# varunagrawal/tiny-faces-pytorch

Measured on AMD Instinct MI355X. Metric: train img/s @ 500x500 bs=12/GPU, higher is better.
Workload: dtype bf16; 1 GPU; configs[2]: bs=12/GPU synthetic 500x500 crops + random boxes; dense_overlap targets on GPU, ResNet-101 hybrid-head fwd, criterion, bwd, fused SGD; global_batch=12, image=500x500, templates=25, parallelism=dp1, weights=random init (tamed kaiming), fp32 master + bf16 MFMA operands

## Files before the change

tiny-faces-pytorch_amd/csrc/common.h:

```cpp
#pragma once
#include <hip/hip_runtime.h>
#include <hip/hip_ext.h>
#include <stdint.h>

#include "../../include/tinyfaces_hip.h"

#define TF_LAUNCH_WITH_STOP_EVENT(kernel, grid, block, lds, stream, ...)                                                  \
  do {                                                                                                                  \
    hipEvent_t ev__ = tf::take_next_stop_event();                                                                       \
    if (ev__) hipExtLaunchKernelGGL(kernel, grid, block, lds, stream, nullptr, ev__, 0, __VA_ARGS__);                   \
    else hipLaunchKernelGGL(kernel, grid, block, lds, stream, __VA_ARGS__);                                             \
  } while (0)

#define TF_LAUNCH_TIMED(kernel, grid, block, lds, stream, ...)                                                            \
  do {                                                                                                                  \
    hipEvent_t f__ = tf::take_next_stop_event(), a__ = nullptr, b__ = nullptr;                                          \
    if (f__) {                                                                                                          \
      tf::ProfScope::fall_back_to_bracket();                                                                            \
      hipExtLaunchKernelGGL(kernel, grid, block, lds, stream, nullptr, f__, 0, __VA_ARGS__);                            \
    } else if (tf::ProfScope::take_launch_events(&a__, &b__)) {                                                         \
      hipExtLaunchKernelGGL(kernel, grid, block, lds, stream, a__, b__, 0, __VA_ARGS__);                                \
    } else {                                                                                                            \
      hipLaunchKernelGGL(kernel, grid, block, lds, stream, __VA_ARGS__);                                                \
    }                                                                                                                   \
  } while (0)

#define TF_CHECK_LAUNCH()                                  \
  do {                                                     \
    hipError_t e__ = hipGetLastError();                    \
    if (e__ != hipSuccess) return TF_ERR_LAUNCH;           \
  } while (0)

namespace tf {

void set_next_stop_event(hipEvent_t e);
hipEvent_t take_next_stop_event();

constexpr int kWave = 64;

__device__ __forceinline__ float bf16_to_f32(uint16_t h) { return __uint_as_float(((uint32_t)h) << 16); }
typedef __bf16 tf_bf16x2 __attribute__((ext_vector_type(2)));
typedef float tf_f32x2 __attribute__((ext_vector_type(2)));
__device__ __forceinline__ uint32_t pack_bf16x2(float lo, float hi) {
  return __builtin_bit_cast(uint32_t, __builtin_convertvector(tf_f32x2{lo, hi}, tf_bf16x2));
}
__device__ __forceinline__ uint16_t f32_to_bf16(float f) { return (uint16_t)(pack_bf16x2(f, 0.f) & 0xffffu); }

template <typename T> struct Elem;
template <> struct Elem<float> {
  static constexpr int kPer16B = 4;
  __device__ static __forceinline__ float load(const float* p) { return *p; }
  __device__ static __forceinline__ void store(float* p, float v) { *p = v; }
};
struct bf16_t { uint16_t v; };
template <> struct Elem<bf16_t> {
  static constexpr int kPer16B = 8;
  __device__ static __forceinline__ float load(const bf16_t* p) { return bf16_to_f32(p->v); }
  __device__ static __forceinline__ void store(bf16_t* p, float v) { p->v = f32_to_bf16(v); }
};

struct f16_t { uint16_t v; };
__device__ __forceinline__ float f16_to_f32(uint16_t h) { return (float)__builtin_bit_cast(_Float16, h); }
__device__ __forceinline__ uint16_t f32_to_f16(float f) { return __builtin_bit_cast(uint16_t, (_Float16)f); }
__device__ __forceinline__ uint32_t pack_f16x2(float lo, float hi) { return (uint32_t)f32_to_f16(lo) | ((uint32_t)f32_to_f16(hi) << 16); }
template <> struct Elem<f16_t> {
  static constexpr int kPer16B = 8;
  __device__ static __forceinline__ float load(const f16_t* p) { return f16_to_f32(p->v); }
  __device__ static __forceinline__ void store(f16_t* p, float v) { p->v = f32_to_f16(v); }
};
template <typename T> __device__ __forceinline__ uint32_t pack2(float lo, float hi);
template <> __device__ __forceinline__ uint32_t pack2<bf16_t>(float lo, float hi) { return pack_bf16x2(lo, hi); }
template <> __device__ __forceinline__ uint32_t pack2<f16_t>(float lo, float hi) { return pack_f16x2(lo, hi); }

template <typename T> __device__ __forceinline__ void unpack16(const uint4& r, float* f);
template <> __device__ __forceinline__ void unpack16<float>(const uint4& r, float* f) {
  f[0] = __uint_as_float(r.x); f[1] = __uint_as_float(r.y); f[2] = __uint_as_float(r.z); f[3] = __uint_as_float(r.w);
}
template <> __device__ __forceinline__ void unpack16<bf16_t>(const uint4& r, float* f) {
  f[0] = __uint_as_float(r.x << 16); f[1] = __uint_as_float(r.x & 0xffff0000u);
  f[2] = __uint_as_float(r.y << 16); f[3] = __uint_as_float(r.y & 0xffff0000u);
  f[4] = __uint_as_float(r.z << 16); f[5] = __uint_as_float(r.z & 0xffff0000u);
  f[6] = __uint_as_float(r.w << 16); f[7] = __uint_as_float(r.w & 0xffff0000u);
}
template <> __device__ __forceinline__ void unpack16<f16_t>(const uint4& r, float* f) {
  f[0] = f16_to_f32((uint16_t)r.x); f[1] = f16_to_f32((uint16_t)(r.x >> 16));
  f[2] = f16_to_f32((uint16_t)r.y); f[3] = f16_to_f32((uint16_t)(r.y >> 16));
  f[4] = f16_to_f32((uint16_t)r.z); f[5] = f16_to_f32((uint16_t)(r.z >> 16));
  f[6] = f16_to_f32((uint16_t)r.w); f[7] = f16_to_f32((uint16_t)(r.w >> 16));
}
template <typename T> __device__ __forceinline__ uint4 pack16(const float* f);
template <> __device__ __forceinline__ uint4 pack16<float>(const float* f) {
  return make_uint4(__float_as_uint(f[0]), __float_as_uint(f[1]), __float_as_uint(f[2]), __float_as_uint(f[3]));
}
template <> __device__ __forceinline__ uint4 pack16<bf16_t>(const float* f) {
  return make_uint4(pack_bf16x2(f[0], f[1]), pack_bf16x2(f[2], f[3]), pack_bf16x2(f[4], f[5]), pack_bf16x2(f[6], f[7]));
}

template <> __device__ __forceinline__ uint4 pack16<f16_t>(const float* f) {
  return make_uint4(pack_f16x2(f[0], f[1]), pack_f16x2(f[2], f[3]), pack_f16x2(f[4], f[5]), pack_f16x2(f[6], f[7]));
}

__device__ __forceinline__ double wave_sum(double v) {
#pragma unroll
  for (int o = 32; o > 0; o >>= 1) v += __shfl_xor(v, o, 64);
  return v;
}
template <int O> __device__ __forceinline__ float lane_xor_sum(float v) {
  if constexpr (O == 8) {
    return v + __int_as_float(__builtin_amdgcn_update_dpp(0, __float_as_int(v), 0x128 , 0xf, 0xf, false));
  } else if constexpr (O == 16) {
    typedef unsigned u32x2_ __attribute__((ext_vector_type(2)));
    const u32x2_ r = __builtin_amdgcn_permlane16_swap(__float_as_uint(v), __float_as_uint(v), false, false);
    return __uint_as_float(r.x) + __uint_as_float(r.y);
  } else if constexpr (O == 32) {
    typedef unsigned u32x2_ __attribute__((ext_vector_type(2)));
    const u32x2_ r = __builtin_amdgcn_permlane32_swap(__float_as_uint(v), __float_as_uint(v), false, false);
    return __uint_as_float(r.x) + __uint_as_float(r.y);
  } else {
    return v + __shfl_xor(v, O, 64);
  }
}
template <int FROM> __device__ __forceinline__ float lane_group_sum(float v) {
  if constexpr (FROM <= 32) { v = lane_xor_sum<FROM>(v); if constexpr (FROM < 32) v = lane_group_sum<FROM * 2>(v); }
  return v;
}
__device__ __forceinline__ float wave_sum(float v) {
  v += __int_as_float(__builtin_amdgcn_update_dpp(0, __float_as_int(v), 0x128, 0xf, 0xf, false));
  v += __int_as_float(__builtin_amdgcn_update_dpp(0, __float_as_int(v), 0x124, 0xf, 0xf, false));
  v += __int_as_float(__builtin_amdgcn_update_dpp(0, __float_as_int(v), 0x122, 0xf, 0xf, false));
  v += __int_as_float(__builtin_amdgcn_update_dpp(0, __float_as_int(v), 0x121, 0xf, 0xf, false));
  return lane_group_sum<16>(v);
}
__device__ __forceinline__ int lane_id() { return threadIdx.x & 63; }

__device__ __host__ __forceinline__ uint64_t mix64(uint64_t z) {
  z += 0x9e3779b97f4a7c15ull;
  z = (z ^ (z >> 30)) * 0xbf58476d1ce4e5b9ull;
  z = (z ^ (z >> 27)) * 0x94d049bb133111ebull;
  return z ^ (z >> 31);
}
__device__ __host__ __forceinline__ uint64_t hash4(uint64_t a, uint64_t b, uint64_t c, uint64_t d) {
  return mix64(mix64(mix64(mix64(a) ^ b) ^ c) ^ d);
}
__device__ __host__ __forceinline__ double u01(uint64_t h) { return (double)(h >> 11) * (1.0 / 9007199254740992.0); }


struct PerDevice {
  bool done[64] = {};
  bool first() { int dev = 0; (void)hipGetDevice(&dev); bool& d = done[dev & 63]; const bool f = !d; d = true; return f; }
};
inline int device_cus() {
  static int cus[64] = {};
  int dev = 0; (void)hipGetDevice(&dev);
  int& n = cus[dev & 63];
  if (n == 0) { int v = 0; if (hipDeviceGetAttribute(&v, hipDeviceAttributeMultiprocessorCount, dev) != hipSuccess || v <= 0) v = 256; n = v; }
  return n;
}

}
```

tiny-faces-pytorch_amd/csrc/targets.hip:

```cpp
#include "targets_shared.h"

namespace {

__device__ __forceinline__ double iou14(double x1, double y1, double x2, double y2, double farea,
                                        double gx1, double gy1, double gx2, double gy2) {
  double bw = gx2 - gx1 + 1.0, bh = gy2 - gy1 + 1.0;
  double barea = bw * bh;
  double xx1 = fmax(x1, gx1), yy1 = fmax(y1, gy1), xx2 = fmin(x2, gx2), yy2 = fmin(y2, gy2);
  double iw = xx2 - xx1 + 1.0, ih = yy2 - yy1 + 1.0;
  double ov = 0.0;
  if (ih > 0.0 && iw > 0.0) {
    double ia = iw * ih;
    double un = farea + barea - ia;
    ov = ia / un;
  }
  return rint(ov * 1e14) / 1e14;
}

__device__ __forceinline__ double noise_at(const TgtParams& p, int b, int flat, int g, int G) {
  if (p.noise) return p.noise[p.noise_off[b] + (int64_t)flat * G + g];
  return tf::u01(tf::hash4(p.seed, (uint64_t)b, (uint64_t)flat, (uint64_t)g));
}

__device__ __forceinline__ bool pad_at(const TgtParams& p, int b, int y, int x, double dx1, double dy1,
                                       double dx2, double dy2) {
  if (!p.paste) return false;
  int xs = (p.flips && p.flips[b]) ? (p.vsx - 1 - x) : x;
  double cx = (double)(p.ofx + xs * p.stx), cy = (double)(p.ofy + y * p.sty);
  const int32_t* pb = p.paste + 4 * b;
  return (cx + dx1 < (double)(pb[0] + 1)) | (cy + dy1 < (double)(pb[1] + 1)) |
         (cx + dx2 > (double)pb[2]) | (cy + dy2 > (double)pb[3]);
}

struct TgtCompParams : TgtParams {
  int32_t* own; double* best; int32_t* count; int32_t* match_count;
  int nslots, N; double T;
};
template <class P> struct is_comp { static constexpr bool value = false; };
template <> struct is_comp<TgtCompParams> { static constexpr bool value = true; };

template <int PHASE, class P = TgtParams>
__global__ void __launch_bounds__(256) targets_kernel(P p) {
  constexpr bool COMP = is_comp<P>::value;
  if constexpr (COMP) {
    if (p.box_off[gridDim.y] > p.nslots) return;
  }
  const int b = blockIdx.y;
  const int cells = p.vsy * p.vsx;
  const int idx = blockIdx.x * 256 + threadIdx.x;
  const bool active = idx < p.nt * cells;
  const int t = active ? idx / cells : 0;
  const int cell = active ? idx - t * cells : 0;
  const int y = cell / p.vsx, x = cell - y * p.vsx;
  const int flat = cell * p.nt + t;
  const int g0 = p.box_off[b], G = p.box_off[b + 1] - g0;
  const double* tp = p.tpl + (size_t)t * p.tstride;
  const double dx1 = tp[0], dy1 = tp[1], dx2 = tp[2], dy2 = tp[3];
  const Anchor an = anchor_at(dx1, dy1, dx2, dy2, p.ofy, p.ofx, p.sty, p.stx, y, x);
  const double fw = an.fw, fh = an.fh;

  double best = -1.0; int bestg = 0;
  for (int g = 0; g < G; ++g) {
    const double* bx = p.boxes + 4 * (size_t)(g0 + g);
    const double gx1 = bx[0], gy1 = bx[1], gx2 = bx[2], gy2 = bx[3];
    double v = -1.0;
    if (active) {
      double r = iou14(an.x1, an.y1, an.x2, an.y2, an.farea, gx1, gy1, gx2, gy2);
      v = r + 1e-6 * noise_at(p, b, flat, g, G);
      if (v > best) { best = v; bestg = g; }
    }
    const bool hot = v > p.neg_thresh;
    if (__ballot(hot)) {
      unsigned long long bits = hot ? (unsigned long long)__double_as_longlong(v) : 0ull;
      if (PHASE == 0) {
        unsigned long long m = bits;
#pragma unroll
        for (int o = 32; o > 0; o >>= 1) {
          unsigned long long other = __shfl_xor(m, o, 64);
          m = other > m ? other : m;
        }
        if (tf::lane_id() == 0) atomicMax(&p.gmax[g0 + g], m);
      } else {
        if (hot && bits == p.gmax[g0 + g]) atomicMin(&p.gidx[g0 + g], (unsigned int)flat);
      }
    }
  }
  if (PHASE != 0 || !active) return;

  float cls = -1.f, tx = 0.f, ty = 0.f, tw = 0.f, th = 0.f;
  if (G > 0) {
    const double* bx = p.boxes + 4 * (size_t)(g0 + bestg);
    const double gx1 = bx[0], gy1 = bx[1], gx2 = bx[2], gy2 = bx[3];
    const double fcx = (gx1 + gx2) / 2.0, fcy = (gy1 + gy2) / 2.0;
    const double coarse_x = (double)(p.ofx + x * p.stx), coarse_y = (double)(p.ofy + y * p.sty);
    tx = (float)((fcx - coarse_x) / fw);
    ty = (float)((fcy - coarse_y) / fh);
    tw = (float)log((gx2 - gx1 + 1.0) / fw);
    th = (float)log((gy2 - gy1 + 1.0) / fh);
    if (best >= p.pos_thresh) cls = 1.f;
    else if (p.neg_thresh <= best && best < p.pos_thresh) cls = 0.f;
  }
  if (cls != -1.f && pad_at(p, b, y, x, dx1, dy1, dx2, dy2)) { cls = 0.f; tx = 0.f; }
  const size_t plane = (size_t)cells;
  p.cls[((size_t)b * p.nt + t) * plane + cell] = cls;
  float* r = p.reg + ((size_t)b * 4 * p.nt + t) * plane + cell;
  r[0] = tx; r[(size_t)p.nt * plane] = ty; r[(size_t)2 * p.nt * plane] = tw; r[(size_t)3 * p.nt * plane] = th;
  if constexpr (COMP) {
    const size_t a = (size_t)b * p.nt * plane + idx;
    p.own[a] = bestg; p.best[a] = best;
  }
}

__global__ void targets_best_anchor_kernel(TgtParams p, int total) {
  int gi = blockIdx.x * blockDim.x + threadIdx.x;
  if (gi >= total) return;
  if (__longlong_as_double((long long)p.gmax[gi]) > p.neg_thresh) {
    const int b = image_of(p.box_off, gi);
    unsigned int flat = p.gidx[gi];
    int t = flat % p.nt, cell = flat / p.nt;
    int y = cell / p.vsx, x = cell - y * p.vsx;
    const double* tp = p.tpl + (size_t)t * p.tstride;
    if (!pad_at(p, b, y, x, tp[0], tp[1], tp[2], tp[3]))
      p.cls[((size_t)b * p.nt + t) * (size_t)(p.vsy * p.vsx) + cell] = 1.f;
  }
}


__global__ void __launch_bounds__(256) targets_count_kernel(TgtCompParams p) {
  if (p.box_off[gridDim.y] > p.nslots) return;
  const int b = blockIdx.y;
  const int A = p.nt * p.vsy * p.vsx;
  const int idx = blockIdx.x * 256 + threadIdx.x;
  int slot = -1;
  if (idx < A) {
    const size_t a = (size_t)b * A + idx;
    if (p.cls[a] == 1.f) slot = p.box_off[b] + p.own[a];
  }
  unsigned long long pending = __ballot(slot >= 0);
  while (pending) {
    const int leader = __ffsll((long long)pending) - 1;
    const int s = __shfl(slot, leader, 64);
    const unsigned long long same = __ballot(slot == s);
    if (tf::lane_id() == leader) atomicAdd(&p.count[s], (int)__popcll(same));
    pending &= ~same;
  }
}

__device__ __forceinline__ bool cand_before(unsigned long long ka, unsigned int fa, unsigned long long kb, unsigned int fb) {
  return ka > kb || (ka == kb && fa < fb);
}

__global__ void __launch_bounds__(256) targets_select_kernel(TgtCompParams p, int B) {
  __shared__ unsigned long long s_k[4];
  __shared__ unsigned int s_f[4];
  const int gi = blockIdx.x;
  const int total = p.box_off[B];
  if (total > p.nslots || gi >= total) return;
  const int cnt = p.count[gi];
  const int need = p.N - cnt;
  if (need <= 0) {
    if (threadIdx.x == 0 && p.match_count) p.match_count[gi] = cnt;
    return;
  }
  const int b = image_of(p.box_off, gi);
  const int g = gi - p.box_off[b];
  const double* bx = p.boxes + 4 * (size_t)gi;
  const double gx1 = bx[0], gy1 = bx[1], gx2 = bx[2], gy2 = bx[3];
  const int cells = p.vsy * p.vsx;
  const size_t img = (size_t)b * p.nt * cells;
  const int wave = threadIdx.x >> 6;
  const double bw = gx2 - gx1 + 1.0, bh = gy2 - gy1 + 1.0, barea = bw * bh;
  const double Tm = p.T - 2e-6;

  unsigned long long prev_k = ~0ull;
  unsigned int prev_f = 0;
  int promoted = 0;
  while (promoted < need) {
    unsigned long long my_k = 0ull;
    unsigned int my_f = 0xffffffffu;
    for (int t = wave; t < p.nt; t += 4) {
      const double* tp = p.tpl + (size_t)t * p.tstride;
      const double dx1 = tp[0], dy1 = tp[1], dx2 = tp[2], dy2 = tp[3];
      const double fw = dx2 - dx1 + 1.0, fh = dy2 - dy1 + 1.0, farea = fw * fh;
      const double larger = fmax(farea, barea);
      if (!(fmin(farea, barea) >= Tm * larger)) continue;
      const double iwm = Tm * larger / fmin(fh, bh) * (1.0 - 1e-9), ihm = Tm * larger / fmin(fw, bw) * (1.0 - 1e-9);
      const double xl = fmax(floor((gx1 - 1.0 + iwm - dx2 - (double)p.ofx) / (double)p.stx), 0.0);
      const double xh = fmin(ceil((gx2 + 1.0 - iwm - dx1 - (double)p.ofx) / (double)p.stx), (double)(p.vsx - 1));
      const double yl = fmax(floor((gy1 - 1.0 + ihm - dy2 - (double)p.ofy) / (double)p.sty), 0.0);
      const double yh = fmin(ceil((gy2 + 1.0 - ihm - dy1 - (double)p.ofy) / (double)p.sty), (double)(p.vsy - 1));
      if (!(xl <= xh) || !(yl <= yh)) continue;
      const int x0 = (int)xl, y0 = (int)yl, ww = (int)xh - x0 + 1, wh = (int)yh - y0 + 1;
      for (int i = tf::lane_id(); i < ww * wh; i += 64) {
        const int wy = i / ww;
        const int y = y0 + wy, x = x0 + (i - wy * ww);
        const int cell = y * p.vsx + x;
        const size_t a = img + (size_t)t * cells + cell;
        if (p.own[a] != g) continue;
        const double bv = p.best[a];
        if (!(bv >= p.T) || p.cls[a] == 1.f || pad_at(p, b, y, x, dx1, dy1, dx2, dy2)) continue;
        const unsigned long long k = (unsigned long long)__double_as_longlong(bv);
        const unsigned int f = (unsigned int)(cell * p.nt + t);
        if (cand_before(prev_k, prev_f, k, f) && cand_before(k, f, my_k, my_f)) { my_k = k; my_f = f; }
      }
    }
#pragma unroll
    for (int o = 32; o > 0; o >>= 1) {
      const unsigned long long ok = __shfl_xor(my_k, o, 64);
      const unsigned int of = __shfl_xor(my_f, o, 64);
      if (cand_before(ok, of, my_k, my_f)) { my_k = ok; my_f = of; }
    }
    if (tf::lane_id() == 0) { s_k[wave] = my_k; s_f[wave] = my_f; }
    __syncthreads();
    unsigned long long win_k = s_k[0];
    unsigned int win_f = s_f[0];
#pragma unroll
    for (int w = 1; w < 4; ++w)
      if (cand_before(s_k[w], s_f[w], win_k, win_f)) { win_k = s_k[w]; win_f = s_f[w]; }
    __syncthreads();
    if (win_k == 0ull) break;
    if (threadIdx.x == 0) {
      const int t = win_f % p.nt, cell = win_f / p.nt;
      p.cls[img + (size_t)t * cells + cell] = 1.f;
    }
    prev_k = win_k; prev_f = win_f;
    ++promoted;
  }
  if (threadIdx.x == 0 && p.match_count) p.match_count[gi] = cnt + promoted;
}

__global__ void iou_dump_kernel(const double* boxes, int G, const double* tpl, int nt, int tstride, int vsy, int vsx,
                                int ofy, int ofx, int sty, int stx, double* out) {
  int flat = blockIdx.x * blockDim.x + threadIdx.x;
  if (flat >= vsy * vsx * nt) return;
  int t = flat % nt, cell = flat / nt, y = cell / vsx, x = cell % vsx;
  const double* tp = tpl + (size_t)t * tstride;
  double cx = (double)ofx + (double)x * ((double)stx / 1.0), cy = (double)ofy + (double)y * ((double)sty / 1.0);
  double fh = tp[3] - tp[1] + 1.0, fw = tp[2] - tp[0] + 1.0;
  for (int g = 0; g < G; ++g)
    out[(size_t)flat * G + g] = iou14(tp[0] + cx, tp[1] + cy, tp[2] + cx, tp[3] + cy, fw * fh,
                                      boxes[4 * g], boxes[4 * g + 1], boxes[4 * g + 2], boxes[4 * g + 3]);
}

}

extern "C" size_t tf_targets_workspace_bytes(int total_boxes) {
  size_t n = (size_t)(total_boxes > 0 ? total_boxes : 1);
  return n * 8 + n * 4 + 64;
}

extern "C" int tf_dense_overlap_targets(const double* boxes, const int32_t* box_offsets, int B,
                                        const double* templates, int nt, int tstride,
                                        int vsy, int vsx, int ofy, int ofx, int sty, int stx,
                                        const int32_t* paste_boxes, const int32_t* flips,
                                        const double* noise, const int64_t* noise_offsets, uint64_t seed,
                                        double pos_thresh, double neg_thresh,
                                        float* class_map, float* reg_map,
                                        void* ws, size_t ws_bytes, void* stream_) {
  hipStream_t stream = (hipStream_t)stream_;
  TgtParams p;
  if (int rc = base_params(p, boxes, box_offsets, B, templates, nt, tstride, vsy, vsx, ofy, ofx, sty, stx, paste_boxes, flips, noise, noise_offsets,
                           seed, pos_thresh, neg_thresh, class_map, reg_map)) return rc;
  size_t nslots = (ws_bytes - 64) / 12;
  if (!ws || ws_bytes < 76) return TF_ERR_WORKSPACE;
  p.gmax = (unsigned long long*)ws;
  p.gidx = (unsigned int*)((char*)ws + nslots * 8);
  if (hipMemsetAsync(p.gmax, 0, nslots * 8, stream) != hipSuccess) return TF_ERR_LAUNCH;
  if (hipMemsetAsync(p.gidx, 0xff, nslots * 4, stream) != hipSuccess) return TF_ERR_LAUNCH;
  dim3 grid((nt * vsy * vsx + 255) / 256, B);
  hipLaunchKernelGGL(targets_kernel<0>, grid, dim3(256), 0, stream, p);
  hipLaunchKernelGGL(targets_kernel<1>, grid, dim3(256), 0, stream, p);
  int total = (int)nslots;
  hipLaunchKernelGGL(targets_best_anchor_kernel, dim3((total + 127) / 128), dim3(128), 0, stream, p, total);
  TF_CHECK_LAUNCH();
  return TF_OK;
}

extern "C" size_t tf_targets_comp_workspace_bytes(int total_boxes, int B, int nt, int vsy, int vsx) {
  size_t n = (size_t)(total_boxes > 0 ? total_boxes : 1);
  size_t anchors = (size_t)(B > 0 ? B : 0) * (size_t)(nt > 0 ? nt : 0) * (size_t)(vsy > 0 ? vsy : 0) * (size_t)(vsx > 0 ? vsx : 0);
  return n * 16 + anchors * 12 + 64;
}

extern "C" int tf_dense_overlap_targets_comp(const double* boxes, const int32_t* box_offsets, int B,
                                             const double* templates, int nt, int tstride,
                                             int vsy, int vsx, int ofy, int ofx, int sty, int stx,
                                             const int32_t* paste_boxes, const int32_t* flips,
                                             const double* noise, const int64_t* noise_offsets, uint64_t seed,
                                             double pos_thresh, double neg_thresh,
                                             int N, double T, int32_t* match_count,
                                             float* class_map, float* reg_map,
                                             void* ws, size_t ws_bytes, void* stream_) {
  hipStream_t stream = (hipStream_t)stream_;
  TgtCompParams p;
  if (int rc = base_params(p, boxes, box_offsets, B, templates, nt, tstride, vsy, vsx, ofy, ofx, sty, stx, paste_boxes, flips, noise, noise_offsets,
                           seed, pos_thresh, neg_thresh, class_map, reg_map)) return rc;
  if (sty <= 0 || stx <= 0) return TF_ERR_ARG;
  if (N < 1 || N > 64) return TF_ERR_ARG;
  if (!(T >= 0.01) || !(T < pos_thresh) || !(T - T == 0.0)) return TF_ERR_ARG;
  const size_t anchors = (size_t)B * nt * vsy * vsx;
  if ((size_t)nt * vsy * vsx > (size_t)0x7fffffff) return TF_ERR_UNSUPPORTED;
  if (!ws || ws_bytes < tf_targets_comp_workspace_bytes(1, B, nt, vsy, vsx)) return TF_ERR_WORKSPACE;
  size_t nslots = (ws_bytes - 64 - anchors * 12) / 16;
  if (nslots > ((size_t)1 << 30)) nslots = (size_t)1 << 30;
  char* w = (char*)ws;
  p.gmax = (unsigned long long*)w;                 w += nslots * 8;
  p.best = (double*)w;                             w += anchors * 8;
  p.gidx = (unsigned int*)w;                       w += nslots * 4;
  p.count = (int32_t*)w;                           w += nslots * 4;
  p.own = (int32_t*)w;
  p.match_count = match_count; p.nslots = (int)nslots; p.N = N; p.T = T;
  if (hipMemsetAsync(p.gmax, 0, nslots * 8, stream) != hipSuccess) return TF_ERR_LAUNCH;
  if (hipMemsetAsync(p.gidx, 0xff, nslots * 4, stream) != hipSuccess) return TF_ERR_LAUNCH;
  if (hipMemsetAsync(p.count, 0, nslots * 4, stream) != hipSuccess) return TF_ERR_LAUNCH;
  dim3 grid((nt * vsy * vsx + 255) / 256, B);
  hipLaunchKernelGGL((targets_kernel<0, TgtCompParams>), grid, dim3(256), 0, stream, p);
  hipLaunchKernelGGL((targets_kernel<1, TgtCompParams>), grid, dim3(256), 0, stream, p);
  const TgtParams& base = p;
  hipLaunchKernelGGL(targets_best_anchor_kernel, dim3(((int)nslots + 127) / 128), dim3(128), 0, stream, base, (int)nslots);
  hipLaunchKernelGGL(targets_count_kernel, grid, dim3(256), 0, stream, p);
  hipLaunchKernelGGL(targets_select_kernel, dim3((unsigned)nslots), dim3(256), 0, stream, p, B);
  TF_CHECK_LAUNCH();
  return TF_OK;
}

extern "C" int tf_dense_overlap_iou(const double* boxes, int G, const double* templates, int nt, int tstride,
                                    int vsy, int vsx, int ofy, int ofx, int sty, int stx,
                                    double* iou_out, void* stream_) {
  if (G <= 0) return TF_OK;
  int n = vsy * vsx * nt;
  hipLaunchKernelGGL(iou_dump_kernel, dim3((n + 255) / 256), dim3(256), 0, (hipStream_t)stream_, boxes, G, templates, nt,
                     tstride, vsy, vsx, ofy, ofx, sty, stx, iou_out);
  TF_CHECK_LAUNCH();
  return TF_OK;
}

namespace {
__global__ void __launch_bounds__(256) pairwise_dist_kernel(const double* __restrict__ boxes, int n, double* __restrict__ out) {
  __shared__ double4 col[256];
  const int j0 = blockIdx.x * 256, i0 = blockIdx.y * 16;
  const int j = j0 + threadIdx.x;
  if (j < n) col[threadIdx.x] = *reinterpret_cast<const double4*>(boxes + 4 * (size_t)j);
  __syncthreads();
  if (j >= n) return;
  const double4 b = col[threadIdx.x];
  const double area_b = (b.z - b.x) * (b.w - b.y);
  for (int i = i0; i < min(n, i0 + 16); ++i) {
    const double4 a = *reinterpret_cast<const double4*>(boxes + 4 * (size_t)i);
    const double area_a = (a.z - a.x) * (a.w - a.y);
    const double xa = fmax(a.x, b.x), ya = fmax(a.y, b.y), xb = fmin(a.z, b.z), yb = fmin(a.w, b.w);
    const double inter = (xb - xa) * (yb - ya);
    const double uni = area_a + area_b - inter;
    out[(size_t)i * n + j] = 1.0 - (uni <= 0.0 ? 0.0 : inter / uni);
  }
}
}

extern "C" int tf_pairwise_iou_distance(const double* boxes, int n, double* out, void* stream) {
  if (n < 0 || (n > 0 && (!boxes || !out))) return TF_ERR_ARG;
  if (n == 0) return TF_OK;
  hipLaunchKernelGGL(pairwise_dist_kernel, dim3((n + 255) / 256, (n + 15) / 16), dim3(256), 0, (hipStream_t)stream, boxes, n, out);
  TF_CHECK_LAUNCH();
  return TF_OK;
}
```

tiny-faces-pytorch_amd/csrc/targets_shared.h:

```cpp
#pragma once
#include "common.h"

namespace {

struct Anchor { double x1, y1, x2, y2, fw, fh, farea; };

__device__ __forceinline__ Anchor anchor_at(double dx1, double dy1, double dx2, double dy2, int ofy, int ofx, int sty, int stx, int y, int x) {
  const double cx = (double)ofx + (double)x * ((double)stx / 1.0);
  const double cy = (double)ofy + (double)y * ((double)sty / 1.0);
  Anchor a;
  a.x1 = dx1 + cx; a.y1 = dy1 + cy; a.x2 = dx2 + cx; a.y2 = dy2 + cy;
  a.fh = dy2 - dy1 + 1.0; a.fw = dx2 - dx1 + 1.0;
  a.farea = a.fw * a.fh;
  return a;
}

__device__ __forceinline__ bool pad_lo(int of, int st, int i, double d1, int lim) { return (double)(of + i * st) + d1 < (double)(lim + 1); }
__device__ __forceinline__ bool pad_hi(int of, int st, int i, double d2, int lim) { return (double)(of + i * st) + d2 > (double)lim; }

__device__ __forceinline__ int clamp_to_int(double v, int lo, int hi) {
  return v >= (double)hi ? hi : (v > (double)lo ? (int)v : lo);
}

__device__ __forceinline__ void unpadded_range(int of, int st, int n, double d1, double d2, int lim_lo, int lim_hi, int& lo, int& hi) {
  lo = clamp_to_int(ceil(((double)(lim_lo + 1) - d1 - (double)of) / (double)st), 0, n);
  while (lo > 0 && !pad_lo(of, st, lo - 1, d1, lim_lo)) --lo;
  while (lo < n && pad_lo(of, st, lo, d1, lim_lo)) ++lo;
  hi = clamp_to_int(floor(((double)lim_hi - d2 - (double)of) / (double)st), -1, n - 1);
  while (hi < n - 1 && !pad_hi(of, st, hi + 1, d2, lim_hi)) ++hi;
  while (hi >= 0 && pad_hi(of, st, hi, d2, lim_hi)) --hi;
}

__device__ __forceinline__ double centre(int of, int st, int i, double d1, double d2) {
  const double c = (double)of + (double)i * ((double)st / 1.0);
  return ((d1 + c) + (d2 + c)) / 2.0;
}
__device__ __forceinline__ double sqdist(int of, int st, int i, double d1, double d2, double fc) {
  const double d = centre(of, st, i, d1, d2) - fc;
  return d * d;
}

__device__ __forceinline__ int nearest_window(int of, int st, int lo, int hi, int w, double d1, double d2, double fc) {
  int c0 = clamp_to_int(floor((fc - (d1 + d2) / 2.0 - (double)of) / (double)st) - (double)(w / 2), lo, hi - w + 1);
  while (c0 > lo && sqdist(of, st, c0 - 1, d1, d2, fc) <= sqdist(of, st, c0 + w - 1, d1, d2, fc)) --c0;
  while (c0 + w <= hi && sqdist(of, st, c0 + w, d1, d2, fc) < sqdist(of, st, c0, d1, d2, fc)) ++c0;
  return c0;
}

__device__ __forceinline__ int image_of(const int32_t* box_off, int gi) {
  int b = 0;
  while (box_off[b + 1] <= gi) ++b;
  return b;
}

struct TgtParams {
  const double* boxes; const int32_t* box_off; const double* tpl; int nt, tstride;
  int vsy, vsx, ofy, ofx, sty, stx;
  const int32_t* paste; const int32_t* flips;
  const double* noise; const int64_t* noise_off; uint64_t seed;
  double pos_thresh, neg_thresh;
  float* cls; float* reg;
  unsigned long long* gmax; unsigned int* gidx;
};

inline int base_params(TgtParams& p, const double* boxes, const int32_t* box_offsets, int B, const double* templates, int nt, int tstride,
                       int vsy, int vsx, int ofy, int ofx, int sty, int stx, const int32_t* paste_boxes, const int32_t* flips,
                       const double* noise, const int64_t* noise_offsets, uint64_t seed, double pos_thresh, double neg_thresh,
                       float* class_map, float* reg_map) {
  if (B <= 0 || nt <= 0 || vsy <= 0 || vsx <= 0 || !box_offsets || !templates || !class_map || !reg_map) return TF_ERR_ARG;
  if (noise && !noise_offsets) return TF_ERR_ARG;
  p.boxes = boxes; p.box_off = box_offsets; p.tpl = templates; p.nt = nt; p.tstride = tstride;
  p.vsy = vsy; p.vsx = vsx; p.ofy = ofy; p.ofx = ofx; p.sty = sty; p.stx = stx;
  p.paste = paste_boxes; p.flips = flips; p.noise = noise; p.noise_off = noise_offsets; p.seed = seed;
  p.pos_thresh = pos_thresh; p.neg_thresh = neg_thresh; p.cls = class_map; p.reg = reg_map;
  return TF_OK;
}

}
```

Before: 1373 img/s.

## Replace second full targets pass with windowed per-box argmax recovery kernel

Removes the PHASE=1 full-grid targets pass and the gidx buffer with its memset. Argmax recovery for each ground-truth box now runs in a per-box block that rescans only the IoU-feasible cell window and recomputes the noisy IoU, keeping the smallest flat index whose value matches gmax. The noise hash is also split so the per-anchor prefix (seed, b, flat) is computed once per anchor instead of per box. This cuts one large kernel launch and redundant IoU work. In exchange it relies on the window bound covering the maximum and on bit-exact recomputation of the value, and it launches one block per workspace slot, most of which exit immediately.

```diff
diff --git a/tiny-faces-pytorch_amd/csrc/common.h b/tiny-faces-pytorch_amd/csrc/common.h
--- a/tiny-faces-pytorch_amd/csrc/common.h
+++ b/tiny-faces-pytorch_amd/csrc/common.h
@@ -139,9 +139,9 @@
   z = (z ^ (z >> 27)) * 0x94d049bb133111ebull;
   return z ^ (z >> 31);
 }
-__device__ __host__ __forceinline__ uint64_t hash4(uint64_t a, uint64_t b, uint64_t c, uint64_t d) {
-  return mix64(mix64(mix64(mix64(a) ^ b) ^ c) ^ d);
-}
+__device__ __host__ __forceinline__ uint64_t hash3(uint64_t a, uint64_t b, uint64_t c) { return mix64(mix64(mix64(a) ^ b) ^ c); }
+__device__ __host__ __forceinline__ uint64_t hash_last(uint64_t key, uint64_t d) { return mix64(key ^ d); }
+__device__ __host__ __forceinline__ uint64_t hash4(uint64_t a, uint64_t b, uint64_t c, uint64_t d) { return hash_last(hash3(a, b, c), d); }
 __device__ __host__ __forceinline__ double u01(uint64_t h) { return (double)(h >> 11) * (1.0 / 9007199254740992.0); }
 
 
diff --git a/tiny-faces-pytorch_amd/csrc/targets.hip b/tiny-faces-pytorch_amd/csrc/targets.hip
--- a/tiny-faces-pytorch_amd/csrc/targets.hip
+++ b/tiny-faces-pytorch_amd/csrc/targets.hip
@@ -8,18 +8,17 @@
   double barea = bw * bh;
   double xx1 = fmax(x1, gx1), yy1 = fmax(y1, gy1), xx2 = fmin(x2, gx2), yy2 = fmin(y2, gy2);
   double iw = xx2 - xx1 + 1.0, ih = yy2 - yy1 + 1.0;
-  double ov = 0.0;
-  if (ih > 0.0 && iw > 0.0) {
-    double ia = iw * ih;
-    double un = farea + barea - ia;
-    ov = ia / un;
-  }
+  if (!(ih > 0.0 && iw > 0.0)) return 0.0;
+  double ia = iw * ih;
+  double un = farea + barea - ia;
+  double ov = ia / un;
   return rint(ov * 1e14) / 1e14;
 }
 
-__device__ __forceinline__ double noise_at(const TgtParams& p, int b, int flat, int g, int G) {
+__device__ __forceinline__ uint64_t noise_key(const TgtParams& p, int b, int flat) { return tf::hash3(p.seed, (uint64_t)b, (uint64_t)flat); }
+__device__ __forceinline__ double noise_at(const TgtParams& p, uint64_t key, int b, int flat, int g, int G) {
   if (p.noise) return p.noise[p.noise_off[b] + (int64_t)flat * G + g];
-  return tf::u01(tf::hash4(p.seed, (uint64_t)b, (uint64_t)flat, (uint64_t)g));
+  return tf::u01(tf::hash_last(key, (uint64_t)g));
 }
 
 __device__ __forceinline__ bool pad_at(const TgtParams& p, int b, int y, int x, double dx1, double dy1,
@@ -39,7 +38,7 @@
 template <class P> struct is_comp { static constexpr bool value = false; };
 template <> struct is_comp<TgtCompParams> { static constexpr bool value = true; };
 
-template <int PHASE, class P = TgtParams>
+template <class P = TgtParams>
 __global__ void __launch_bounds__(256) targets_kernel(P p) {
   constexpr bool COMP = is_comp<P>::value;
   if constexpr (COMP) {
@@ -58,6 +57,7 @@
   const double dx1 = tp[0], dy1 = tp[1], dx2 = tp[2], dy2 = tp[3];
   const Anchor an = anchor_at(dx1, dy1, dx2, dy2, p.ofy, p.ofx, p.sty, p.stx, y, x);
   const double fw = an.fw, fh = an.fh;
+  const uint64_t key = noise_key(p, b, flat);
 
   double best = -1.0; int bestg = 0;
   for (int g = 0; g < G; ++g) {
@@ -66,26 +66,21 @@
     double v = -1.0;
     if (active) {
       double r = iou14(an.x1, an.y1, an.x2, an.y2, an.farea, gx1, gy1, gx2, gy2);
-      v = r + 1e-6 * noise_at(p, b, flat, g, G);
+      v = r + 1e-6 * noise_at(p, key, b, flat, g, G);
       if (v > best) { best = v; bestg = g; }
     }
     const bool hot = v > p.neg_thresh;
     if (__ballot(hot)) {
-      unsigned long long bits = hot ? (unsigned long long)__double_as_longlong(v) : 0ull;
-      if (PHASE == 0) {
-        unsigned long long m = bits;
+      unsigned long long m = hot ? (unsigned long long)__double_as_longlong(v) : 0ull;
 #pragma unroll
-        for (int o = 32; o > 0; o >>= 1) {
-          unsigned long long other = __shfl_xor(m, o, 64);
-          m = other > m ? other : m;
-        }
-        if (tf::lane_id() == 0) atomicMax(&p.gmax[g0 + g], m);
-      } else {
-        if (hot && bits == p.gmax[g0 + g]) atomicMin(&p.gidx[g0 + g], (unsigned int)flat);
+      for (int o = 32; o > 0; o >>= 1) {
+        unsigned long long other = __shfl_xor(m, o, 64);
+        m = other > m ? other : m;
       }
-    }
-  }
-  if (PHASE != 0 || !active) return;
+      if (tf::lane_id() == 0) atomicMax(&p.gmax[g0 + g], m);
+    }
+  }
+  if (!active) return;
 
   float cls = -1.f, tx = 0.f, ty = 0.f, tw = 0.f, th = 0.f;
   if (G > 0) {
@@ -111,18 +106,49 @@
   }
 }
 
-__global__ void targets_best_anchor_kernel(TgtParams p, int total) {
-  int gi = blockIdx.x * blockDim.x + threadIdx.x;
-  if (gi >= total) return;
-  if (__longlong_as_double((long long)p.gmax[gi]) > p.neg_thresh) {
-    const int b = image_of(p.box_off, gi);
-    unsigned int flat = p.gidx[gi];
-    int t = flat % p.nt, cell = flat / p.nt;
-    int y = cell / p.vsx, x = cell - y * p.vsx;
+__global__ void __launch_bounds__(256) targets_best_anchor_kernel(TgtParams p, int B, int nslots) {
+  __shared__ unsigned int s_f[4];
+  const int gi = blockIdx.x;
+  const int total = p.box_off[B];
+  if (total > nslots || gi >= total) return;
+  const unsigned long long m = p.gmax[gi];
+  const double mv = __longlong_as_double((long long)m);
+  if (!(mv > p.neg_thresh)) return;
+  const int b = image_of(p.box_off, gi);
+  const int g0 = p.box_off[b], g = gi - g0, G = p.box_off[b + 1] - g0;
+  const double* bx = p.boxes + 4 * (size_t)gi;
+  const double gx1 = bx[0], gy1 = bx[1], gx2 = bx[2], gy2 = bx[3];
+  const double Tm = (mv - mv == 0.0 ? mv : p.neg_thresh) - 2e-6;
+  const int wave = threadIdx.x >> 6;
+
+  unsigned int my_f = 0xffffffffu;
+  for (int t = wave; t < p.nt; t += 4) {
     const double* tp = p.tpl + (size_t)t * p.tstride;
-    if (!pad_at(p, b, y, x, tp[0], tp[1], tp[2], tp[3]))
-      p.cls[((size_t)b * p.nt + t) * (size_t)(p.vsy * p.vsx) + cell] = 1.f;
-  }
+    const double dx1 = tp[0], dy1 = tp[1], dx2 = tp[2], dy2 = tp[3];
+    CellWindow w;
+    if (!iou_window(Tm, dx1, dy1, dx2, dy2, gx1, gy1, gx2, gy2, p.ofy, p.ofx, p.sty, p.stx, p.vsy, p.vsx, w)) continue;
+    for (int i = tf::lane_id(); i < w.ww * w.wh; i += 64) {
+      const int wy = i / w.ww;
+      const int y = w.y0 + wy, x = w.x0 + (i - wy * w.ww);
+      const int flat = (y * p.vsx + x) * p.nt + t;
+      const Anchor an = anchor_at(dx1, dy1, dx2, dy2, p.ofy, p.ofx, p.sty, p.stx, y, x);
+      const double r = iou14(an.x1, an.y1, an.x2, an.y2, an.farea, gx1, gy1, gx2, gy2);
+      const double v = r + 1e-6 * noise_at(p, noise_key(p, b, flat), b, flat, g, G);
+      if ((unsigned long long)__double_as_longlong(v) == m) my_f = min(my_f, (unsigned int)flat);
+    }
+  }
+#pragma unroll
+  for (int o = 32; o > 0; o >>= 1) my_f = min(my_f, (unsigned int)__shfl_xor(my_f, o, 64));
+  if (tf::lane_id() == 0) s_f[wave] = my_f;
+  __syncthreads();
+  if (threadIdx.x != 0) return;
+  const unsigned int flat = min(min(s_f[0], s_f[1]), min(s_f[2], s_f[3]));
+  if (flat == 0xffffffffu) return;
+  const int t = flat % p.nt, cell = flat / p.nt;
+  const int y = cell / p.vsx, x = cell - y * p.vsx;
+  const double* tp = p.tpl + (size_t)t * p.tstride;
+  if (!pad_at(p, b, y, x, tp[0], tp[1], tp[2], tp[3]))
+    p.cls[((size_t)b * p.nt + t) * (size_t)(p.vsy * p.vsx) + cell] = 1.f;
 }
 
 
@@ -169,7 +195,6 @@
   const int cells = p.vsy * p.vsx;
   const size_t img = (size_t)b * p.nt * cells;
   const int wave = threadIdx.x >> 6;
-  const double bw = gx2 - gx1 + 1.0, bh = gy2 - gy1 + 1.0, barea = bw * bh;
   const double Tm = p.T - 2e-6;
 
   unsigned long long prev_k = ~0ull;
@@ -181,19 +206,11 @@
     for (int t = wave; t < p.nt; t += 4) {
       const double* tp = p.tpl + (size_t)t * p.tstride;
       const double dx1 = tp[0], dy1 = tp[1], dx2 = tp[2], dy2 = tp[3];
-      const double fw = dx2 - dx1 + 1.0, fh = dy2 - dy1 + 1.0, farea = fw * fh;
-      const double larger = fmax(farea, barea);
-      if (!(fmin(farea, barea) >= Tm * larger)) continue;
-      const double iwm = Tm * larger / fmin(fh, bh) * (1.0 - 1e-9), ihm = Tm * larger / fmin(fw, bw) * (1.0 - 1e-9);
-      const double xl = fmax(floor((gx1 - 1.0 + iwm - dx2 - (double)p.ofx) / (double)p.stx), 0.0);
-      const double xh = fmin(ceil((gx2 + 1.0 - iwm - dx1 - (double)p.ofx) / (double)p.stx), (double)(p.vsx - 1));
-      const double yl = fmax(floor((gy1 - 1.0 + ihm - dy2 - (double)p.ofy) / (double)p.sty), 0.0);
-      const double yh = fmin(ceil((gy2 + 1.0 - ihm - dy1 - (double)p.ofy) / (double)p.sty), (double)(p.vsy - 1));
-      if (!(xl <= xh) || !(yl <= yh)) continue;
-      const int x0 = (int)xl, y0 = (int)yl, ww = (int)xh - x0 + 1, wh = (int)yh - y0 + 1;
-      for (int i = tf::lane_id(); i < ww * wh; i += 64) {
-        const int wy = i / ww;
-        const int y = y0 + wy, x = x0 + (i - wy * ww);
+      CellWindow w;
+      if (!iou_window(Tm, dx1, dy1, dx2, dy2, gx1, gy1, gx2, gy2, p.ofy, p.ofx, p.sty, p.stx, p.vsy, p.vsx, w)) continue;
+      for (int i = tf::lane_id(); i < w.ww * w.wh; i += 64) {
+        const int wy = i / w.ww;
+        const int y = w.y0 + wy, x = w.x0 + (i - wy * w.ww);
         const int cell = y * p.vsx + x;
         const size_t a = img + (size_t)t * cells + cell;
         if (p.own[a] != g) continue;
@@ -263,15 +280,12 @@
                            seed, pos_thresh, neg_thresh, class_map, reg_map)) return rc;
   size_t nslots = (ws_bytes - 64) / 12;
   if (!ws || ws_bytes < 76) return TF_ERR_WORKSPACE;
+  if (nslots > ((size_t)1 << 30)) nslots = (size_t)1 << 30;
   p.gmax = (unsigned long long*)ws;
-  p.gidx = (unsigned int*)((char*)ws + nslots * 8);
   if (hipMemsetAsync(p.gmax, 0, nslots * 8, stream) != hipSuccess) return TF_ERR_LAUNCH;
-  if (hipMemsetAsync(p.gidx, 0xff, nslots * 4, stream) != hipSuccess) return TF_ERR_LAUNCH;
   dim3 grid((nt * vsy * vsx + 255) / 256, B);
-  hipLaunchKernelGGL(targets_kernel<0>, grid, dim3(256), 0, stream, p);
-  hipLaunchKernelGGL(targets_kernel<1>, grid, dim3(256), 0, stream, p);
-  int total = (int)nslots;
-  hipLaunchKernelGGL(targets_best_anchor_kernel, dim3((total + 127) / 128), dim3(128), 0, stream, p, total);
+  hipLaunchKernelGGL(targets_kernel<TgtParams>, grid, dim3(256), 0, stream, p);
+  hipLaunchKernelGGL(targets_best_anchor_kernel, dim3((unsigned)nslots), dim3(256), 0, stream, p, B, (int)nslots);
   TF_CHECK_LAUNCH();
   return TF_OK;
 }
@@ -306,18 +320,16 @@
   char* w = (char*)ws;
   p.gmax = (unsigned long long*)w;                 w += nslots * 8;
   p.best = (double*)w;                             w += anchors * 8;
-  p.gidx = (unsigned int*)w;                       w += nslots * 4;
+  w += nslots * 4;
   p.count = (int32_t*)w;                           w += nslots * 4;
   p.own = (int32_t*)w;
   p.match_count = match_count; p.nslots = (int)nslots; p.N = N; p.T = T;
   if (hipMemsetAsync(p.gmax, 0, nslots * 8, stream) != hipSuccess) return TF_ERR_LAUNCH;
-  if (hipMemsetAsync(p.gidx, 0xff, nslots * 4, stream) != hipSuccess) return TF_ERR_LAUNCH;
   if (hipMemsetAsync(p.count, 0, nslots * 4, stream) != hipSuccess) return TF_ERR_LAUNCH;
   dim3 grid((nt * vsy * vsx + 255) / 256, B);
-  hipLaunchKernelGGL((targets_kernel<0, TgtCompParams>), grid, dim3(256), 0, stream, p);
-  hipLaunchKernelGGL((targets_kernel<1, TgtCompParams>), grid, dim3(256), 0, stream, p);
+  hipLaunchKernelGGL(targets_kernel<TgtCompParams>, grid, dim3(256), 0, stream, p);
   const TgtParams& base = p;
-  hipLaunchKernelGGL(targets_best_anchor_kernel, dim3(((int)nslots + 127) / 128), dim3(128), 0, stream, base, (int)nslots);
+  hipLaunchKernelGGL(targets_best_anchor_kernel, dim3((unsigned)nslots), dim3(256), 0, stream, base, B, (int)nslots);
   hipLaunchKernelGGL(targets_count_kernel, grid, dim3(256), 0, stream, p);
   hipLaunchKernelGGL(targets_select_kernel, dim3((unsigned)nslots), dim3(256), 0, stream, p, B);
   TF_CHECK_LAUNCH();
diff --git a/tiny-faces-pytorch_amd/csrc/targets_shared.h b/tiny-faces-pytorch_amd/csrc/targets_shared.h
--- a/tiny-faces-pytorch_amd/csrc/targets_shared.h
+++ b/tiny-faces-pytorch_amd/csrc/targets_shared.h
@@ -47,6 +47,26 @@
   return c0;
 }
 
+struct CellWindow { int x0, y0, ww, wh; };
+
+__device__ __forceinline__ bool iou_window(double Tm, double dx1, double dy1, double dx2, double dy2, double gx1, double gy1, double gx2, double gy2,
+                                           int ofy, int ofx, int sty, int stx, int vsy, int vsx, CellWindow& w) {
+  w.x0 = 0; w.y0 = 0; w.ww = vsx; w.wh = vsy;
+  if (!(Tm > 0.0) || sty <= 0 || stx <= 0) return true;
+  const double bw = gx2 - gx1 + 1.0, bh = gy2 - gy1 + 1.0, barea = bw * bh;
+  const double fw = dx2 - dx1 + 1.0, fh = dy2 - dy1 + 1.0, farea = fw * fh;
+  const double larger = fmax(farea, barea);
+  if (!(fmin(farea, barea) >= Tm * larger)) return false;
+  const double iwm = Tm * larger / fmin(fh, bh) * (1.0 - 1e-9), ihm = Tm * larger / fmin(fw, bw) * (1.0 - 1e-9);
+  const double xl = fmax(floor((gx1 - 1.0 + iwm - dx2 - (double)ofx) / (double)stx), 0.0);
+  const double xh = fmin(ceil((gx2 + 1.0 - iwm - dx1 - (double)ofx) / (double)stx), (double)(vsx - 1));
+  const double yl = fmax(floor((gy1 - 1.0 + ihm - dy2 - (double)ofy) / (double)sty), 0.0);
+  const double yh = fmin(ceil((gy2 + 1.0 - ihm - dy1 - (double)ofy) / (double)sty), (double)(vsy - 1));
+  if (!(xl <= xh) || !(yl <= yh)) return false;
+  w.x0 = (int)xl; w.y0 = (int)yl; w.ww = (int)xh - w.x0 + 1; w.wh = (int)yh - w.y0 + 1;
+  return true;
+}
+
 __device__ __forceinline__ int image_of(const int32_t* box_off, int gi) {
   int b = 0;
   while (box_off[b + 1] <= gi) ++b;
@@ -60,7 +80,7 @@
   const double* noise; const int64_t* noise_off; uint64_t seed;
   double pos_thresh, neg_thresh;
   float* cls; float* reg;
-  unsigned long long* gmax; unsigned int* gidx;
+  unsigned long long* gmax;
 };
 
 inline int base_params(TgtParams& p, const double* boxes, const int32_t* box_offsets, int B, const double* templates, int nt, int tstride,
```

Measured after the change: 1379 img/s (median of 6 runs). Within noise of the previous version (+0.4%).
